# laurits-mumberg/kube-scheduler-simulator-p9

Measured on AMD Instinct MI355X. Metric: filter+score pod x node pairs/sec (5k nodes, Fit+BalancedAllocation), higher is better.
Workload: dtype int64+f64; 1 GPU; cfg2: 5,000 nodes x 10,000 pods, NodeResourcesFit+NodeResourcesBalancedAllocation; nodes_per_gpu=5000, nodes_total=5000, pods=10000, parallelism=1 GPU

## Files before the change

kube-scheduler-simulator-p9_amd/csrc/engine.hip:

```cpp
#include <hip/hip_runtime.h>

#include <algorithm>
#include <cmath>
#include <cstdlib>
#include <cstring>
#include <memory>
#include <string>
#include <vector>
#include <utility>
#include <deque>
#include <atomic>
#include <map>
#include <mutex>
#include <chrono>
#include <cstddef>
#include <thread>

#include "engine.h"
#include <rccl/rccl.h>

namespace ksg {

#define HIPCHK(x)                                                                 \
  do {                                                                            \
// ... 3502 lines not shown
  static_assert(96 * 4 + sizeof(PodLite) + 16 <= 192 * 4, "eval LDS layout");
  auto fetch = [&](uint32_t kk, RowV& r, StaticRec& sr, bool loaded) {
    const uint32_t to = kk * KSG_TILE + tid, nn = tile * A.tile_len + to;
    if (to < A.tile_len && nn < C.N) {
      const int hit = pend_lds((int32_t)(C.goff + nn));
      if (hit >= 0) r = ld_obj<PER>(&A.pprev[hit].after);
      else if (!loaded) load_row_p<PER>(C, nn, A.need_eph, r);
      if (STAT) sr = srec_at<PER>(A, q, C.goff + nn);
    }
  };
  StaticRec snext{KSG_FILTER_PASS, 0};
  fetch(0, rnext, snext, true);
#pragma unroll 1
  for (uint32_t k = 0; k < A.npt; ++k) {
  KSG_ETIME(t0);
  if (A.estamps && w == 15) asm volatile("s_waitcnt vmcnt(0)" ::: "memory");
  KSG_ETIME(tl);
  t_wait += tl - t0;
  const uint32_t to = k * KSG_TILE + tid, n = tile * A.tile_len + to;
  const RowV r = rnext;
  const StaticRec sr = snext;
  if (k + 1 < A.npt) fetch(k + 1, rnext, snext, false);
  uint64_t key = 0;
  bool feasible = false, achT = false, achA = false;
  if (to < A.tile_len && n < C.N) {
    int32_t fit_s, ba_s;
    int64_t total;
    uint32_t code, raw = 0;
    if (STAT) {
      const int64_t MT = mlds[0], MA = mlds[1];
      code = eval_row_s<MODE>(r, F, h, C.R < 4 ? C.R : 4, sr, MT, MA, fit_s, ba_s, total);
      raw = sr.raw;
      achT = F.pos_taint >= 0 && (int64_t)(raw >> 20) == MT;
      achA = F.pos_na >= 0 && !(h->flags & KPF_SKIP_NA_SCORE) && (int64_t)(raw & KSG_RAW_NA_MASK) == MA;
    } else {
      code = eval_row<MODE>(r, F, h, C.R < 4 ? C.R : 4, fit_s, ba_s, total);
    }
    if (stash_all || w == 0) {
      stash[(stash_all ? k * 16 + w : k) * 64 + lane] = PatchV{code, fit_s | (ba_s << 16), (int32_t)total, raw};
    } else {
      uint32_t* of;
      int32_t *os, *ot;
      out_ptrs(A, q, C.N, of, os, ot);
      if (PER && kept_q(A, q)) write_pair<STAT, true>(F, of, os, ot, C.N, n, code, fit_s, ba_s, total, raw);
      else write_pair<STAT, false>(F, of, os, ot, C.N, n, code, fit_s, ba_s, total, raw);
    }
    if (code == KSG_FILTER_PASS) {
      feasible = true;
      key = pack_key(total, F.seed, h->queue_idx, C.goff + n);
    }
  }
  cF += (uint32_t)__popcll(__ballot(feasible));
  if (STAT) {
    cT += (uint32_t)__popcll(__ballot(feasible && achT));
    cA += (uint32_t)__popcll(__ballot(feasible && achA));
  }
  KSG_ETIME(t1);
  key = wave_sort_desc(key);
  top = k == 0 ? key : wave_merge_top(top, wave_reverse(key));
  KSG_ETIME(t2);
  t_eval += t1 - t0;
  t_sort += t2 - t1;
  }
  KSG_ETIME(t3);
  L[w * 64 + lane] = top;
  if (lane == 0) {
    wcount[w] = cF;
    wcount[32 + w] = cT;
    wcount[48 + w] = cA;
  }
  lds_barrier();
#pragma unroll 1
  for (int s = 8; s >= 1; s >>= 1) {
    if (w < s) L[w * 64 + lane] = wave_merge_top(L[w * 64 + lane], L[(w + s) * 64 + 63 - lane]);
    lds_barrier();
  }
  if (w == 0) {
    uint64_t* dst = A.tile_top + ((size_t)b * A.T + tile) * KSG_TOPK;
    __hip_atomic_store(dst + lane, L[lane], __ATOMIC_RELAXED, __HIP_MEMORY_SCOPE_AGENT);
    if (lane < 3) {
      const int off = lane == 0 ? 0 : 16 + 16 * lane;
      int32_t c = 0;
      for (int k = 0; k < 16; ++k) c += (int32_t)wcount[off + k];
      __hip_atomic_store(A.tile_feas + ((size_t)b * A.T + tile) * 3 + lane, c, __ATOMIC_RELAXED,
                         __HIP_MEMORY_SCOPE_AGENT);
    }
    asm volatile("s_waitcnt vmcnt(0)" ::: "memory");
    uint32_t old = 0;
    if (lane == 0) old = __hip_atomic_fetch_add(A.arrive + b * A.astride, 1u, __ATOMIC_RELAXED, __HIP_MEMORY_SCOPE_AGENT);
    old = __builtin_amdgcn_readfirstlane(old);
    if (lane == 0) wcount[16] = old == A.T - 1 ? 1u : 0u;
  }
  auto flush_stash = [&]() {
    if (!stash_all && w != 0) return;
    uint32_t* of;
    int32_t *os, *ot;
    out_ptrs(A, q, C.N, of, os, ot);
#pragma unroll 1
    for (uint32_t k = 0; k < A.npt; ++k) {
      const uint32_t to = k * KSG_TILE + tid, n = tile * A.tile_len + to;
      if (to >= A.tile_len || n >= C.N) break;
      const PatchV pt = stash[(stash_all ? k * 16 + w : k) * 64 + lane];
      if (PER && kept_q(A, q)) write_pair<STAT, true>(F, of, os, ot, C.N, n, pt.code, pt.fitba & 0xFFFF, pt.fitba >> 16, pt.total, pt.raw);
      else write_pair<STAT, false>(F, of, os, ot, C.N, n, pt.code, pt.fitba & 0xFFFF, pt.fitba >> 16, pt.total, pt.raw);
    }
  };
  auto signal_flushed = [&]() {
    if constexpr (PER) {
      asm volatile("s_waitcnt vmcnt(0)" ::: "memory");
      __syncthreads();
      if (tid == 0) __hip_atomic_fetch_add(A.flushed, 1u, __ATOMIC_RELAXED, __HIP_MEMORY_SCOPE_AGENT);
    }
  };
  lds_barrier();
  KSG_ETIME(t4);
#undef KSG_ETIME
  if (est) {
    atomicAdd((unsigned long long*)&A.estamps[13], (unsigned long long)t_eval);
    atomicAdd((unsigned long long*)&A.estamps[14], (unsigned long long)t_sort);
    atomicAdd((unsigned long long*)&A.estamps[15], (unsigned long long)(t4 - t3));
    atomicAdd((unsigned long long*)&A.estamps[18], (unsigned long long)t_wait);
  }
  if (A.estamps && tid == 0) {
    __builtin_amdgcn_sched_barrier(0);
    const uint64_t t = __builtin_amdgcn_s_memrealtime();
    __builtin_amdgcn_sched_barrier(0);
    atomicMax((unsigned long long*)&A.estamps[9], (unsigned long long)t);
    atomicMax((unsigned long long*)&A.estamps[28], (unsigned long long)(t - t_start));
    atomicAdd((unsigned long long*)&A.estamps[29], (unsigned long long)(t - t_start));
    atomicAdd((unsigned long long*)&A.estamps[31], 1ull);
  }
  if (!wcount[16]) {
    flush_stash();
    signal_flushed();
    return;
  }
  win_merge<PER>(C, A, b, L, pnl, np);
  flush_stash();
  signal_flushed();
}

struct SumLite {
  uint64_t best_key;
  int32_t selected, feasible, status, pad;
};
struct Delta {
  int64_t req[4];
  int64_t nzc, nzm;
  int32_t pods;
};
#define KSG_HSLOTS 128
struct PickTab {
  int32_t node[KSG_HSLOTS];
  int32_t first[KSG_HSLOTS], last[KSG_HSLOTS], cnt[KSG_HSLOTS];
};
struct WinLDS {
  uint64_t key[KSG_BATCH][KSG_CAND];
  RowV row[KSG_BATCH][KSG_STAGE];
  Pend prior[KSG_BATCH];
  PodLite pod[KSG_BATCH];
  PatchV patch[KSG_BATCH][KSG_CAND];
  uint64_t pkey[KSG_BATCH][KSG_BATCH];
  int8_t pdf[KSG_BATCH][KSG_BATCH];
  uint64_t pmask[KSG_BATCH];
  uint32_t nxt_ok;
  uint64_t pbest[KSG_BATCH];
  int32_t pbest_e[KSG_BATCH];
  int32_t S[3][KSG_BATCH];
  int32_t O[3][KSG_BATCH];
  int32_t feas[KSG_BATCH];
  SumLite sum[KSG_BATCH];
  int32_t ptn[KSG_HSLOTS], pte[KSG_HSLOTS];
  int32_t gtn[KSG_HSLOTS], gtf[KSG_HSLOTS];
  PickTab pick[3];
  uint64_t kc[KSG_BATCH][KSG_CAND];
  uint64_t rk[KSG_BATCH][KSG_BATCH];
  int8_t rdf[KSG_BATCH][KSG_BATCH];
  int32_t pf[KSG_BATCH];
  int32_t achT[KSG_BATCH], achA[KSG_BATCH];
  int64_t mt[KSG_BATCH], ma[KSG_BATCH];
  int64_t xmt[KSG_BATCH], xma[KSG_BATCH];
  int8_t pdfT[KSG_BATCH][KSG_BATCH], pdfA[KSG_BATCH][KSG_BATCH];
  int8_t rdfT[KSG_BATCH][KSG_BATCH], rdfA[KSG_BATCH][KSG_BATCH];
  int32_t fbf[KSG_BATCH];
  uint64_t red[16][4];
};

static_assert(sizeof(WinLDS) <= 160 * 1024, "window LDS exceeds the CU's 160 KiB");
static constexpr uint32_t kStashNpt =
    (uint32_t)std::min<size_t>(KSG_STASH_NPT, (sizeof(WinLDS) - (16 * 64 * 8 + 192 * 4)) / (16 * 64 * sizeof(PatchV)));
static_assert(kStashNpt >= 1, "eval blocks' output stash exceeds the window LDS");
__device__ __forceinline__ uint32_t hslot(int32_t node) { return ((uint32_t)node * 2654435761u) >> 25; }
__device__ __forceinline__ int prior_of(const WinLDS& L, int32_t x) {
  uint32_t h = hslot(x);
  for (int k = 0; k < KSG_HSLOTS; ++k) {
    int32_t v = L.ptn[h];
    if (v == x) return L.pte[h];
    if (v == -1) return -1;
    h = (h + 1) & (KSG_HSLOTS - 1);
  }
  return -1;
}
__device__ __forceinline__ uint32_t tab_claim(int32_t* nodes, int32_t x) {
  uint32_t h = hslot(x);
  for (int k = 0; k < KSG_HSLOTS; ++k) {
    int32_t old = atomicCAS(&nodes[h], -1, x);
    if (old == -1 || old == x) return h;
    h = (h + 1) & (KSG_HSLOTS - 1);
  }
  return 0;
}
__device__ __forceinline__ int tab_find(const int32_t* nodes, int32_t x) {
  uint32_t h = hslot(x);
  for (int k = 0; k < KSG_HSLOTS; ++k) {
    int32_t v = nodes[h];
    if (v == x) return (int)h;
    if (v == -1) return -1;
    h = (h + 1) & (KSG_HSLOTS - 1);
  }
  return -1;
}
__device__ __forceinline__ void pick_insert(PickTab& T, int32_t x, int b) {
  uint32_t h = tab_claim(T.node, x);
  atomicMin(&T.first[h], b);
  atomicMax(&T.last[h], b);
  atomicAdd(&T.cnt[h], 1);
}
__device__ __forceinline__ void pick_clear(PickTab& T, int i) {
  T.node[i] = -1;
  T.first[i] = KSG_BATCH;
  T.last[i] = -1;
  T.cnt[i] = 0;
}
__device__ __forceinline__ int first_pick(const PickTab& T, int32_t x) {
  int h = x >= 0 ? tab_find(T.node, x) : -1;
  return h >= 0 ? T.first[h] : KSG_BATCH;
}

#define KSG_ORG_NODE 0x40000000
template <bool PER = false>
__device__ __forceinline__ void origin_rows(const DevCluster& C, const WinLDS& L, const WinArgs& A, int32_t o,
                                            RowV& start, RowV& snap) {
  if (o & KSG_ORG_NODE) {
    if (A.xrows) start = A.xrows[o & 0xFFFFF];
    else load_row(C, (uint32_t)(o & 0xFFFFF) - C.goff, A.need_eph, start);
    snap = start;
  } else if (o < KSG_BATCH) {
    start = L.prior[o].after;
    snap = L.prior[o].base;
  } else {
    int p = (o - 64) >> 6, i = (o - 64) & 63;
    if (i < KSG_STAGE) start = L.row[p][i];
    else if (PER) load_row_p<PER>(C, (uint32_t)(L.key[p][i] & 0xFFFFFull) - C.goff, A.need_eph, start);
    else start = rec_rows(A.wrec)[p * KSG_CAND + i];
    snap = start;
  }
}
__device__ __forceinline__ void delta_of(const PodLite& p, Delta& d) {
#pragma unroll
  for (int k = 0; k < 4; ++k) d.req[k] = p.req[k];
  d.nzc = p.nz_cpu;
  d.nzm = p.nz_mem;
  d.pods = 1;
}
__device__ __forceinline__ void delta_add(Delta& d, const PodLite& p) {
#pragma unroll
  for (int k = 0; k < 4; ++k) d.req[k] += p.req[k];
  d.nzc += p.nz_cpu;
  d.nzm += p.nz_mem;
  d.pods += 1;
}
__device__ __forceinline__ void apply_delta(RowV& r, const Delta& d, uint32_t R) {
#pragma unroll
  for (uint32_t k = 0; k < 4; ++k)
    if (k < R) r.req[k] += d.req[k];
  r.nzc += d.nzc;
  r.nzm += d.nzm;
  r.podcnt += d.pods;
}
__device__ __forceinline__ void pick_chain(const WinLDS& L, const int32_t* S, int a, int32_t x, Delta& cum, int& nx) {
  cum = Delta{};
  nx = KSG_BATCH;
  for (int j = 0; j < KSG_BATCH; ++j)
    if (S[j] == x) {
      if (j <= a) delta_add(cum, L.pod[j]);
      else if (nx == KSG_BATCH) nx = j;
    }
}
__device__ __forceinline__ uint64_t max3u(uint64_t a, uint64_t b, uint64_t c) {
  uint64_t m = a > b ? a : b;
  return m > c ? m : c;
}

template <bool PER = false>
__device__ __forceinline__ void row_under(const DevCluster& C, const WinLDS& L, const WinArgs& A, const int32_t* S,
                                          const PickTab& T, int b, uint32_t gu, uint32_t R, RowV& r) {
  const int32_t g = (int32_t)gu;
  const int e = prior_of(L, g);
  if (e >= 0) r = L.prior[e].after;
  else if (A.xrows) r = A.xrows[g];
  else load_row_p<PER>(C, gu - C.goff, A.need_eph, r);
  const int hs = tab_find(T.node, g);
  if (hs >= 0 && T.first[hs] < b) {
    Delta cum{};
    for (int j = 0; j < b; ++j)
      if (S[j] == g) delta_add(cum, L.pod[j]);
    apply_delta(r, cum, R);
  }
}
template <int MODE, bool PER = false>
__device__ __forceinline__ void win_exact_select(const DevCluster& C, const DevProfile& F, const WinArgs& A, WinLDS& L,
                                              int b, int cur, int nxt, uint32_t R) {
  const int tid = threadIdx.x, lane = tid & 63, wave = tid >> 6;
  const PodLite* h = &L.pod[b];
  const int32_t* S = L.S[cur];
  const PickTab& T = L.pick[cur];
  const uint32_t g0 = A.xrows ? 0u : C.goff, gn = A.xrows ? A.G : C.N;
  int32_t feas = 0;
  int64_t lt = 0, la = 0;
#pragma unroll 1
  for (uint32_t i = tid; i < gn; i += KSG_WIN_THREADS) {
    RowV r;
    row_under<PER>(C, L, A, S, T, b, g0 + i, R, r);
    const StaticRec sr = srec_at<PER>(A, A.w0 + b, g0 + i);
    int32_t fs, bs;
    int64_t tot;
    if (eval_row_s<MODE>(r, F, h, R, sr, 0, 0, fs, bs, tot) == KSG_FILTER_PASS) {
      ++feas;
      lt = max(lt, (int64_t)(sr.raw >> 20));
      la = max(la, (int64_t)(sr.raw & KSG_RAW_NA_MASK));
    }
  }
  feas = wave_sum(feas);
  lt = wave_max(lt);
  la = wave_max(la);
  if (lane == 0) {
    L.red[wave][0] = (uint64_t)feas;
    L.red[wave][1] = (uint64_t)lt;
    L.red[wave][2] = (uint64_t)la;
  }
  lds_barrier();
  int32_t fa = 0;
  int64_t mt = 0, ma = 0;
  for (int w = 0; w < KSG_WIN_THREADS / 64; ++w) {
    fa += (int32_t)L.red[w][0];
    mt = max(mt, (int64_t)L.red[w][1]);
    ma = max(ma, (int64_t)L.red[w][2]);
  }
  uint64_t best = 0;
#pragma unroll 1
  for (uint32_t i = tid; i < gn; i += KSG_WIN_THREADS) {
    RowV r;
    row_under<PER>(C, L, A, S, T, b, g0 + i, R, r);
    int32_t fs, bs;
    int64_t tot;
    if (eval_row_s<MODE>(r, F, h, R, srec_at<PER>(A, A.w0 + b, g0 + i), mt, ma, fs, bs, tot) == KSG_FILTER_PASS) {
      const uint64_t k = pack_key(tot, F.seed, h->queue_idx, g0 + i);
      best = k > best ? k : best;
    }
  }
  best = wave_max(best);
  if (lane == 0) L.red[wave][3] = best;
  lds_barrier();
  if (tid == 0) {
    uint64_t bk = 0;
    for (int w = 0; w < KSG_WIN_THREADS / 64; ++w) bk = L.red[w][3] > bk ? L.red[w][3] : bk;
    const int32_t sel = (fa > 0 && bk) ? (int32_t)(bk & 0xFFFFFull) : -1;
    int32_t org = -1;
    if (sel >= 0) {
      const int e = prior_of(L, sel);
      org = e >= 0 ? e : (KSG_ORG_NODE | sel);
      pick_insert(L.pick[nxt], sel, b);
    }
    L.S[nxt][b] = sel;
    L.O[nxt][b] = org;
    SumLite& sm = L.sum[b];
    sm.best_key = sel >= 0 ? (fa == 1 ? (bk & 0xFFFFFFFFFFull) : bk) : 0;
    sm.selected = sel;
    sm.feasible = fa;
    sm.status = sel >= 0 ? 0 : 1;
    L.xmt[b] = mt;
    L.xma[b] = (h->flags & KPF_SKIP_NA_SCORE) ? 0 : ma;
  }
}
template <int MODE, bool PER = false>
__device__ __forceinline__ void win_exact_write(const DevCluster& C, const DevProfile& F, const WinArgs& A, WinLDS& L,
                                             int b, int cur, uint32_t R) {
  const PodLite* h = &L.pod[b];
  uint32_t* of;
  int32_t *os, *ot;
  out_ptrs(A, A.w0 + b, C.N, of, os, ot);
  const int64_t mt = L.xmt[b], ma = L.xma[b];
#pragma unroll 1
  for (uint32_t i = threadIdx.x; i < C.N; i += KSG_WIN_THREADS) {
    RowV r;
    row_under<PER>(C, L, A, L.S[cur], L.pick[cur], b, C.goff + i, R, r);
    const StaticRec sr = srec_at<PER>(A, A.w0 + b, C.goff + i);
    int32_t fs, bs;
    int64_t tot;
    const uint32_t code = eval_row_s<MODE>(r, F, h, R, sr, mt, ma, fs, bs, tot);
    if (PER && kept_q(A, A.w0 + b)) write_pair<true, true>(F, of, os, ot, C.N, i, code, fs, bs, tot, sr.raw);
    else write_pair<true>(F, of, os, ot, C.N, i, code, fs, bs, tot, sr.raw);
  }
}

template <int MODE, bool STAT, bool PER = false>
__device__ __forceinline__ void win_fixup(const DevCluster& C, const DevProfile& F, const WinArgs& A, WinLDS& L) {
  int tid_ = (int)threadIdx.x;
#ifndef KSG_FIXUP_HOIST
  asm volatile("" : "+v"(tid_));
#endif
  const int tid = tid_, lane = tid & 63, wave = tid >> 6;
  const int nb = (int)A.nw;
  const uint32_t R = C.R < 4 ? C.R : 4;
#define STAMP(k)                                        \
  if (A.stamps && tid == 0) {                           \
    __builtin_amdgcn_sched_barrier(0);                  \
    A.stamps[k] = __builtin_amdgcn_s_memtime();         \
    __builtin_amdgcn_sched_barrier(0);                  \
  }
  STAMP(0);
  if (A.stamps && tid == 0) A.stamps[11] = __builtin_amdgcn_s_memrealtime();
  const bool p_late = PER && A.pub_wait != nullptr;
  int np = 0;
  int32_t pn_all = -1;
  uint64_t pv = 0;
  constexpr int kRowW = (int)(sizeof(RowV) / 8), kPendW = (int)(sizeof(Pend) / 8);
  auto p_loads = [&]() {
    np = ldv<PER>(A.pprev_n);
    pn_all = wave == 0 && lane < KSG_BATCH ? ldv<PER>(&A.pprev[lane].node) : -1;
  };
  auto p_list_load = [&]() {
    pv = tid < KSG_BATCH * kPendW ? ldv<PER>(reinterpret_cast<const uint64_t*>(A.pprev) + tid) : 0;
  };
  if (!p_late) p_loads();
  const uint64_t* keys = rec_keys(A.wrec);
  const uint64_t* rows = reinterpret_cast<const uint64_t*>(rec_rows(A.wrec));
  const int nk = nb * KSG_CAND, nr = nb * KSG_STAGE * kRowW;
  uint64_t kv[2], rv[6];
  const ShallowRows* SR = shallow_rows(A.wrec);
// ... 26 lines not shown
    auto small_stores = [&]() {
      if (tid < nb * kPodW) reinterpret_cast<uint64_t*>(L.pod)[tid] = qv;
      if (tid < nb) L.feas[tid] = fv;
      if (STAT && tid < nb) {
        L.achT[tid] = aT;
        L.achA[tid] = aA;
        L.mt[tid] = m0;
        L.ma[tid] = m1;
        L.fbf[tid] = 0;
      }
      if (tid < 3 * KSG_BATCH) {
        (&L.S[0][0])[tid] = -1;
        (&L.O[0][0])[tid] = -1;
      }
      if (tid < KSG_HSLOTS) {
#pragma unroll
        for (int t = 0; t < 3; ++t) pick_clear(L.pick[t], tid);
      }
    };
    if (p_late) small_stores();
    if (p_late) {
      if (tid == 0) {
        bool ok = false;
        if (A.rstamps) A.rstamps[0] = __builtin_amdgcn_s_memrealtime();
        for (uint32_t it = 0; it < A.spin; ++it) {
          if (ld_sc1(A.pub_wait) >= A.pub_wait_need) { ok = true; break; }
          if ((it & 63u) == 63u && ld_sc1(A.abortw) != 0u) break;
          __builtin_amdgcn_s_sleep(1);
        }
        if (A.rstamps) A.rstamps[1] = __builtin_amdgcn_s_memrealtime();
        if (!ok) __hip_atomic_store(A.abortw, 1u, __ATOMIC_RELAXED, __HIP_MEMORY_SCOPE_AGENT);
      }
      lds_barrier();
      p_loads();
      p_list_load();
    }
    if (tid < np * kPendW) reinterpret_cast<uint64_t*>(L.prior)[tid] = pv;
    if (!p_late) small_stores();
    if (wave == 0) {
      const int32_t pnode = lane < np ? pn_all : -1;
      L.ptn[lane] = -1;
      L.ptn[lane + 64] = -1;
      if (lane < np) L.pte[tab_claim(L.ptn, pnode)] = lane;
    }
  }
  lds_barrier();
  STAMP(1);
  if (tid < np) {
    const Pend& pe = L.prior[tid];
    uint32_t nl = (uint32_t)pe.node - C.goff;
    if ((uint32_t)pe.node >= C.goff && nl < C.N) store_row_p<PER>(C, nl, pe.after);
    if (A.xrows) A.xrows[pe.node] = pe.after;
  }
  {
    const int pb = 2 * wave + (lane >> 5), e = lane & 31;
    uint64_t k = 0;
    if (pb < nb && e < np) {
      const Pend& pe = L.prior[e];
      const PodLite* h = &L.pod[pb];
      int32_t fs, bs;
      int64_t tot;
      StaticRec sr{KSG_FILTER_PASS, 0};
      uint32_t code;
      if (STAT) {
        sr = srec_at<PER>(A, A.w0 + pb, (uint32_t)pe.node);
        code = eval_row_s<MODE>(pe.after, F, h, R, sr, L.mt[pb], L.ma[pb], fs, bs, tot);
      } else {
        code = eval_row<MODE>(pe.after, F, h, R, fs, bs, tot);
      }
      bool snap_ok = sr.code == KSG_FILTER_PASS && (F.pos_fit < 0 || fit_filter_row(pe.base, h, R) == 0);
      PatchV pt;
      pt.code = code;
      pt.fitba = fs | (bs << 16);
      pt.total = (int32_t)tot;
      pt.raw = sr.raw;
      L.patch[pb][e] = pt;
      k = code == KSG_FILTER_PASS ? pack_key(tot, F.seed, h->queue_idx, (uint32_t)pe.node) : 0;
      L.pkey[pb][e] = k;
      const int df = (code == KSG_FILTER_PASS ? 1 : 0) - (snap_ok ? 1 : 0);
      L.pdf[pb][e] = (int8_t)df;
      if (STAT) {
        const bool na_on = F.pos_na >= 0 && !(h->flags & KPF_SKIP_NA_SCORE);
        L.pdfT[pb][e] = (int8_t)(F.pos_taint >= 0 && (int64_t)(sr.raw >> 20) == L.mt[pb] ? df : 0);
        L.pdfA[pb][e] = (int8_t)(na_on && (int64_t)(sr.raw & KSG_RAW_NA_MASK) == L.ma[pb] ? df : 0);
      }
    }
    STAMP(16);
    uint64_t k0 = wave_max(lane < 32 ? k : (uint64_t)0), k1 = wave_max(lane >= 32 ? k : (uint64_t)0);
    unsigned long long m0 = __ballot(k0 && lane < 32 && k == k0), m1 = __ballot(k1 && lane >= 32 && k == k1);
    if (lane == 0) {
      if (2 * wave < nb) {
        L.pbest[2 * wave] = k0;
        L.pbest_e[2 * wave] = m0 ? __ffsll((long long)m0) - 1 : -1;
      }
      if (2 * wave + 1 < nb) {
        L.pbest[2 * wave + 1] = k1;
        L.pbest_e[2 * wave + 1] = m1 ? __ffsll((long long)m1) - 1 - 32 : -1;
      }
    }
  }
#pragma unroll
  for (int k = 0; k < 2; ++k) {
    int i = tid + k * KSG_WIN_THREADS;
    if (i < nk) (&L.key[0][0])[i] = kv[k];
    const int b = wave + 16 * k;
    bool m = kv[k] != 0 && np > 0 && prior_of(L, (int32_t)(kv[k] & 0xFFFFFull)) >= 0;
    unsigned long long mask = __ballot(m);
    if (lane == 0 && b < nb) L.pmask[b] = mask;
  }
#pragma unroll
  for (int k = 0; k < 6; ++k) {
    int i = tid + k * KSG_WIN_THREADS;
    if (i < nr) reinterpret_cast<uint64_t*>(&L.row[0][0])[i] = rv[k];
  }
  lds_barrier();
  STAMP(17);
  STAMP(2);
  if (wave == 0) {
    const int b = lane;
    const bool valid = b < nb;
    const uint64_t pm = valid ? L.pmask[b] : 0;
    const uint64_t pbk = valid ? L.pbest[b] : 0;
    int r = 0;
    bool pok = pbk != 0;
    int32_t node = -1, org = -1;
#pragma unroll 1
    for (int round = 0; round < 64; ++round) {
      uint64_t ck = 0;
      if (valid) {
        uint64_t free_ = ~pm & (r < 64 ? (~0ull << r) : 0ull);
        r = free_ ? __ffsll((long long)free_) - 1 : KSG_CAND;
        ck = r < KSG_CAND ? L.key[b][r] : 0;
      }
      uint64_t pk = pok ? pbk : 0;
      uint64_t best = ck > pk ? ck : pk;
      bool from_c = best != 0 && best == ck;
      node = best ? (int32_t)(best & 0xFFFFFull) : -1;
      org = !best ? -1 : from_c ? 64 + b * 64 + r : L.pbest_e[b];
      L.gtn[lane] = -1;
      L.gtn[lane + 64] = -1;
      uint32_t h = 0;
      if (node >= 0) {
        h = tab_claim(L.gtn, node);
        L.gtf[h] = KSG_BATCH;
      }
      if (node >= 0) atomicMin(&L.gtf[h], b);
      bool lose = node >= 0 && L.gtf[h] < b;
      if (__ballot(lose) == 0) break;
      if (lose) {
        if (from_c) ++r;
        else pok = false;
      }
    }
    if (valid) {
      L.S[0][b] = node;
      L.O[0][b] = org;
      if (node >= 0) pick_insert(L.pick[0], node, b);
    }
  }
  lds_barrier();
  STAMP(3);
  int cur = 0, stable = 0;
  uint32_t iters = 0;
#pragma unroll 1
  for (;;) {
    const int nxt = cur == 2 ? 0 : cur + 1;
    if (tid < KSG_HSLOTS) pick_clear(L.pick[nxt == 2 ? 0 : nxt + 1], tid);
    const PickTab& T = L.pick[cur];
    if (wave < 8) {
      const int p_hi = nb * (nb - 1) / 2;
#pragma unroll 1
      for (int base = stable * (stable - 1) / 2 + wave * 64; base < p_hi; base += 8 * 64) {
        const int p = base + lane;
        if (p < p_hi) {
          int b = (int)((1.0f + sqrtf(1.0f + 8.0f * (float)p)) * 0.5f);
          b = b * (b - 1) / 2 > p ? b - 1 : ((b + 1) * b / 2 <= p ? b + 1 : b);
          const int a = p - b * (b - 1) / 2;
          const int32_t Sv = L.S[cur][a];
          uint64_t k = 0;
          int df = 0, dT = 0, dA = 0;
          PatchV pt;
          pt.code = KSG_NOT_PATCHED;
          pt.fitba = pt.total = 0;
          pt.raw = 0;
          if (Sv >= 0) {
            int nx = KSG_BATCH;
            Delta cum;
            delta_of(L.pod[a], cum);
            if (iters == 0) STAMP(24);
            if (T.cnt[tab_find(T.node, Sv)] > 1) pick_chain(L, L.S[cur], a, Sv, cum, nx);
            if (iters == 0) STAMP(25);
            if (nx >= b) {
              RowV cur_r, snap;
              origin_rows<PER>(C, L, A, L.O[cur][a], cur_r, snap);
              apply_delta(cur_r, cum, R);
              const PodLite* h = &L.pod[b];
              int32_t fs, bs;
              int64_t tot;

              StaticRec sr{KSG_FILTER_PASS, 0};
              uint32_t code;
              if (STAT) {
                sr = srec_at<PER>(A, A.w0 + b, (uint32_t)Sv);
                code = eval_row_s<MODE>(cur_r, F, h, R, sr, L.mt[b], L.ma[b], fs, bs, tot);
              } else {
                code = eval_row<MODE>(cur_r, F, h, R, fs, bs, tot);
              }

              bool snap_ok = sr.code == KSG_FILTER_PASS && (F.pos_fit < 0 || fit_filter_row(snap, h, R) == 0);
              df = (code == KSG_FILTER_PASS ? 1 : 0) - (snap_ok ? 1 : 0);
              if (STAT) {
                const bool na_on = F.pos_na >= 0 && !(h->flags & KPF_SKIP_NA_SCORE);
                dT = F.pos_taint >= 0 && (int64_t)(sr.raw >> 20) == L.mt[b] ? df : 0;
                dA = na_on && (int64_t)(sr.raw & KSG_RAW_NA_MASK) == L.ma[b] ? df : 0;
              }
              if (code == KSG_FILTER_PASS) k = pack_key(tot, F.seed, h->queue_idx, (uint32_t)Sv);
              pt.code = code;
              pt.fitba = fs | (bs << 16);
              pt.total = (int32_t)tot;
              pt.raw = sr.raw;
            }
          }
          L.rk[b][a] = k;
          L.rdf[b][a] = (int8_t)df;
          if (STAT) {
            L.rdfT[b][a] = (int8_t)dT;
            L.rdfA[b][a] = (int8_t)dA;
          }
          L.patch[b][32 + a] = pt;
        }
      }
    } else {
      if (wave == 8 && lane < np) L.pf[lane] = first_pick(T, L.prior[lane].node);
#pragma unroll 1
      for (int b = stable + (wave - 8); b < nb; b += 8) {
        const uint64_t ck = L.key[b][lane];
        const bool mod = ((L.pmask[b] >> lane) & 1) || (ck != 0 && first_pick(T, (int32_t)(ck & 0xFFFFFull)) < b);
        L.kc[b][lane] = mod ? 0 : ck;
      }
    }
    if (iters == 0) STAMP(21);
    lds_barrier();
    if (iters == 0) STAMP(22);
#pragma unroll 1
    for (int hh = 0; hh < 2; ++hh) {
      const int b = 2 * wave + hh;
      if (b >= nb) break;
      if (b < stable) {
        if (lane == 0) {
          int32_t s = L.S[cur][b];
          L.S[nxt][b] = s;
          L.O[nxt][b] = L.O[cur][b];
          if (s >= 0) pick_insert(L.pick[nxt], s, b);
        }
        continue;
      }
      const bool pact = lane < np && L.pf[lane & 31] >= b;
      const uint64_t kc = L.kc[b][lane];
      const uint64_t kp = pact ? L.pkey[b][lane & 31] : 0;
      const uint64_t kr = lane < b ? L.rk[b][lane & 31] : 0;
      const int df = (pact ? (int)L.pdf[b][lane & 31] : 0) + (lane < b ? (int)L.rdf[b][lane & 31] : 0);
      const uint64_t best = wave_max(max3u(kc, kp, kr));
      int feasible;
      bool fb = false;
      if (STAT) {
        const int dT = (pact ? (int)L.pdfT[b][lane & 31] : 0) + (lane < b ? (int)L.rdfT[b][lane & 31] : 0);
        const int dA = (pact ? (int)L.pdfA[b][lane & 31] : 0) + (lane < b ? (int)L.rdfA[b][lane & 31] : 0);
        const int sum = wave_sum((df + 2) | ((dT + 2) << 10) | ((dA + 2) << 20));
        feasible = L.feas[b] + (sum & 1023) - 128;
        const int achT = L.achT[b] + ((sum >> 10) & 1023) - 128, achA = L.achA[b] + ((sum >> 20) & 1023) - 128;
        const bool na_on = F.pos_na >= 0 && !(L.pod[b].flags & KPF_SKIP_NA_SCORE);
        fb = !(L.pod[b].flags & KPF_PREFILTER_ERROR) && !na_prescore_error(L.pod[b].flags, feasible) && feasible > 0 &&
             ((F.pos_taint >= 0 && achT <= 0) || (na_on && achA <= 0));
      } else {
        feasible = L.feas[b] + wave_sum(df);
      }
      const bool perr = (L.pod[b].flags & KPF_PREFILTER_ERROR) != 0 || na_prescore_error(L.pod[b].flags, feasible);
      const int32_t sel = (feasible > 0 && best && !perr) ? (int32_t)(best & 0xFFFFFull) : -1;
      const unsigned long long mc = __ballot(best && kc == best), mp = __ballot(best && kp == best),
                               mr = __ballot(best && kr == best);
      if (STAT && lane == 0) L.fbf[b] = fb ? 1 : 0;
      if (fb) continue;
      if (lane == 0) {
        if (STAT) {
          L.xmt[b] = L.mt[b] < 0 ? 0 : L.mt[b];
          L.xma[b] = (F.pos_na < 0 || (L.pod[b].flags & KPF_SKIP_NA_SCORE) || L.ma[b] < 0) ? 0 : L.ma[b];
        }
        int32_t org = -1;
        if (mc) org = 64 + b * 64 + (__ffsll((long long)mc) - 1);
        else if (mp) org = __ffsll((long long)mp) - 1;
        else if (mr) org = L.O[cur][__ffsll((long long)mr) - 1];
        L.S[nxt][b] = sel;
        L.O[nxt][b] = sel >= 0 ? org : -1;
        if (sel >= 0) pick_insert(L.pick[nxt], sel, b);
        SumLite& sm = L.sum[b];
        sm.best_key = sel >= 0 ? (feasible == 1 ? (best & 0xFFFFFFFFFFull) : best) : 0;
        sm.selected = sel;
        sm.feasible = feasible;
        sm.status = perr ? 2 : (sel >= 0 ? 0 : 1);
      }
    }
    if (iters == 0) STAMP(23);
    lds_barrier();
    if (STAT) {
      unsigned long long fm = __ballot(lane < nb && lane >= stable && L.fbf[lane & 31] != 0);
      if (fm) {
        while (fm) {
          const int b = __ffsll((long long)fm) - 1;
          fm &= fm - 1;
          win_exact_select<MODE, PER>(C, F, A, L, b, cur, nxt, R);
        }
        lds_barrier();
      }
    }
    if (iters < 2) STAMP(19 + iters);
    ++iters;
    {
      const int32_t so = L.S[cur][lane & 31], sn = L.S[nxt][lane & 31];
      unsigned long long m = __ballot(lane < nb && lane >= stable && sn != so);
      stable = m ? min(__ffsll((long long)m), nb) : nb;
    }
    cur = nxt;
    if (stable >= nb) break;
  }
  STAMP(4);
  if (A.stamps && tid == 0) A.stamps[7] = iters;
  uint32_t pre_fl = 0, pre_ev = 0;
  if (PER && tid == 0) {
    pre_fl = ld_sc1(A.flushed);
    pre_ev = A.nxt_evd ? ld_sc1(A.nxt_evd) : 0u;
  }
  auto flushed_wait = [&]() {
    if (tid == 0) {
      bool ok = pre_fl >= A.flush_need;
      for (uint32_t it = 0; !ok && it < A.spin; ++it) {
        if (ld_sc1(A.flushed) >= A.flush_need) { ok = true; break; }
        if ((it & 63u) == 63u && ld_sc1(A.abortw) != 0u) break;
        __builtin_amdgcn_s_sleep(2);
      }
      if (!ok) __hip_atomic_store(A.abortw, 1u, __ATOMIC_RELAXED, __HIP_MEMORY_SCOPE_AGENT);
    }
    lds_barrier();
  };
  auto exact_writes = [&]() {
    unsigned long long fm = __ballot(lane < nb && L.fbf[lane & 31] != 0);
    while (fm) {
      const int b = __ffsll((long long)fm) - 1;
      fm &= fm - 1;
      win_exact_write<MODE, PER>(C, F, A, L, b, cur, R);
    }
  };
  bool exact_early = false;
  if constexpr (PER && STAT) {
    if (A.replay2 && __ballot(lane < nb && L.fbf[lane & 31] != 0) != 0) {
      exact_early = true;
      flushed_wait();
      exact_writes();
    }
  }
  const PickTab& T = L.pick[cur];
  if (wave == 0) {
    const int a = lane;
    const int32_t Sv = a < nb ? L.S[cur][a] : -1;
    int h = Sv >= 0 ? tab_find(T.node, Sv) : -1;
    const bool last = h >= 0 && T.last[h] == a;
    unsigned long long m = __ballot(last);
    if (last) {
      Delta cum;
      delta_of(L.pod[a], cum);
      int nx;
      if (T.cnt[h] > 1) pick_chain(L, L.S[cur], a, Sv, cum, nx);
      RowV st, snap;
      origin_rows<PER>(C, L, A, L.O[cur][a], st, snap);
      Pend p;
      p.node = Sv;
      p.pad = 0;
      p.base = st;
      apply_delta(st, cum, R);
      p.after = st;
      st_obj<PER>(A.pnext + __popcll(m & ((1ull << a) - 1)), p);
    }
    if (lane == 0) stv<PER>(A.pnext_n, (int32_t)__popcll(m));
  }
  STAMP(26);
  if constexpr (PER) {
    asm volatile("s_waitcnt vmcnt(0)" ::: "memory");
    STAMP(27);
    __syncthreads();
    if (tid < 16) {
      if (A.replay2) __hip_atomic_fetch_max(A.pub + tid * 32, A.pub_val, __ATOMIC_RELAXED, __HIP_MEMORY_SCOPE_AGENT);
      else st_sc1(A.pub + tid * 32, A.pub_val);
    }
    if (A.rstamps && tid == 0) A.rstamps[2] = __builtin_amdgcn_s_memrealtime();
  }
  STAMP(6);
  if (tid < nb) {
    ksg_pod_summary& d = A.sums[A.w0 + tid];
    d.best_key = L.sum[tid].best_key;
    d.selected = L.sum[tid].selected;
    d.feasible = L.sum[tid].feasible;
    d.status = L.sum[tid].status;
    if (STAT) {
      if (F.pos_taint >= 0) d.max_score[F.pos_taint] = L.xmt[tid];
      if (F.pos_na >= 0) d.max_score[F.pos_na] = L.xma[tid];
    }
  }
  if constexpr (PER) {
    if (tid == 0) L.nxt_ok = A.nxt_evd && pre_ev >= A.nxt_need ? 1u : 0u;
    if (!exact_early) flushed_wait();
  }
  {
    const int32_t Sv = L.S[cur][lane & 31];
    const int32_t pn = lane < np ? L.prior[lane].node : -1;
    const int pf = lane < np ? first_pick(T, pn) : -1;
#pragma unroll 1
    for (int hh = 0; hh < 2; ++hh) {
      const int b = 2 * wave + hh;
      if (b >= nb) break;
      if (STAT && L.fbf[b]) continue;
      const PatchV pt = L.patch[b][lane];
      const bool wr = lane < 32 ? (lane < np && pf >= b) : (lane - 32 < b && pt.code != KSG_NOT_PATCHED);
      const int32_t node = lane < 32 ? pn : Sv;
      const uint32_t nl = (uint32_t)node - C.goff;
      if (wr && node >= 0 && (uint32_t)node >= C.goff && nl < C.N) {
        uint32_t* of;
        int32_t *os, *ot;
        out_ptrs(A, A.w0 + b, C.N, of, os, ot);
        if (PER && kept_q(A, A.w0 + b))
          write_pair<STAT, true>(F, of, os, ot, C.N, nl, pt.code, pt.fitba & 0xFFFF, pt.fitba >> 16, pt.total, pt.raw);
        else
          write_pair<STAT, false>(F, of, os, ot, C.N, nl, pt.code, pt.fitba & 0xFFFF, pt.fitba >> 16, pt.total, pt.raw);
      }
    }
  }
  if (STAT && !exact_early) exact_writes();
  STAMP(5);
  if (A.stamps && tid == 0) A.stamps[12] = __builtin_amdgcn_s_memrealtime();
#undef STAMP
}

template <int MODE, bool STAT>
__global__ __launch_bounds__(KSG_WIN_THREADS) void k_window(DevCluster C, DevProfile F, WinArgs A) {
  extern __shared__ __attribute__((aligned(16))) unsigned char lds_raw[];
  uint32_t warm = 0;
  KWarm<0, (int)((sizeof(DevCluster) + sizeof(DevProfile) + sizeof(WinArgs)) / 64 * 64)>::run(
      (const void*)__builtin_amdgcn_kernarg_segment_ptr(), warm);
  warm_wait(warm);
  if (blockIdx.x == 0) {
    if (A.nw) win_fixup<MODE, STAT>(C, F, A, *reinterpret_cast<WinLDS*>(lds_raw));
    return;
  }
  win_eval<MODE, STAT>(C, F, A, blockIdx.x - 1, reinterpret_cast<uint64_t*>(lds_raw));
}

__global__ void k_apply_pend(DevCluster C, const Pend* p, const int32_t* pn) {
  int e = threadIdx.x;
  if (e >= *pn) return;
  uint32_t nl = (uint32_t)p[e].node - C.goff;
  if ((uint32_t)p[e].node >= C.goff && nl < C.N) store_row(C, nl, p[e].after);
}

__global__ __launch_bounds__(64) void k_window_gmerge(const uint8_t* recv, uint32_t ranks, const RowV* xrows,
                                                      const Pend* pl, const int32_t* pn, uint8_t* out) {
  __shared__ uint64_t keys[8 * KSG_CAND];
  const uint32_t b = blockIdx.x;
  const int lane = threadIdx.x;
  for (uint32_t r = 0; r < ranks; ++r) keys[r * KSG_CAND + lane] = rec_keys(recv + r * kXchgBytes)[(size_t)b * KSG_CAND + lane];
  __syncthreads();
  uint64_t v = keys[lane];
  for (uint32_t r = 1; r < ranks; ++r) v = wave_merge_top(v, keys[r * KSG_CAND + 63 - lane]);
  int32_t f[3] = {0, 0, 0};
  for (uint32_t r = 0; r < ranks; ++r)
    for (int k = 0; k < 3; ++k) f[k] += reinterpret_cast<const int32_t*>(recv + r * kXchgBytes)[k * KSG_BATCH + b];
  RowV c;
  memset(&c, 0, sizeof(c));
  if (v) {
    const int32_t gid = (int32_t)(v & 0xFFFFFull);
    const int np = *pn;
    int hit = -1;
    for (int e = 0; e < np; ++e) hit = pl[e].node == gid ? e : hit;
    c = hit >= 0 ? pl[hit].after : xrows[gid];
  }
  rec_keys(out)[(size_t)b * KSG_CAND + lane] = v;
  rec_rows(out)[(size_t)b * KSG_CAND + lane] = c;
  if (lane < 3) reinterpret_cast<int32_t*>(out)[lane * KSG_BATCH + b] = f[lane];
}
__global__ void k_rows_pack(DevCluster C, uint32_t need_eph, RowV* out) {
  const uint32_t n = blockIdx.x * blockDim.x + threadIdx.x;
  if (n < C.N) load_row(C, n, need_eph, out[n]);
}
__global__ void k_rows_unpack(const RowV* recv, uint32_t ranks, uint32_t G, uint32_t stride, RowV* xrows) {
  const uint32_t r = blockIdx.y;
  const uint32_t lo = (uint32_t)((uint64_t)G * r / ranks), hi = (uint32_t)((uint64_t)G * (r + 1) / ranks);
  for (uint32_t i = blockIdx.x * blockDim.x + threadIdx.x; lo + i < hi; i += gridDim.x * blockDim.x)
    xrows[lo + i] = recv[(size_t)r * stride + i];
}

#include "table_chain.hip"

struct WinSync {
  uint32_t replayed[16][32];
  uint32_t evd[2];
  uint32_t pad1[30];
  uint32_t flushed[2];
  uint32_t pad2[30];
};
struct WinRunArgs {
  uint32_t nwin, first, count, T;
  uint32_t tt_sz, tf_sz;
  uint64_t* tile_top;
  int32_t* tfeas;
  uint8_t* wrec;
  Pend* pend;
  int32_t* pend_n;
  uint32_t* arrive;
  uint64_t* stamps;
  const uint32_t* sready;
  uint32_t sready_need;
};
__device__ bool win_stat_gate(const WinRunArgs& R, uint32_t r0, uint32_t n, uint32_t* abortw, uint32_t spin,
                              uint32_t* go) {
  if (threadIdx.x == 0) {
    const uint32_t g0 = r0 / KSG_SD_PODS, g1 = (r0 + n - 1) / KSG_SD_PODS;
    bool ok = false;
    for (uint32_t it = 0; it < spin; ++it) {
      bool all = true;
      for (uint32_t g = g0; g <= g1; ++g) all &= ld_sc1(R.sready + g) >= R.sready_need;
      if (all) { ok = true; break; }
      if ((it & 63u) == 63u && ld_sc1(abortw) != 0u) break;
      __builtin_amdgcn_s_sleep(2);
    }
    if (!ok) __hip_atomic_store(abortw, 1u, __ATOMIC_RELAXED, __HIP_MEMORY_SCOPE_AGENT);
// ... 3170 lines not shown
```

Baseline: 8.209 billion pairs/s.

## Cache per-pick base/after rows in LDS across fixpoint iterations

Adds a per-batch PickRow cache in LDS holding base, after and snap rows plus the next-pick index for each selected node. Each pairwise conflict evaluation and the final pending-row output now read these cached rows instead of rebuilding them through origin_rows and pick_chain on every pair. The change also drops the last/cnt atomics from the pick table, specializes the non-STAT selection path with paired wave reductions, and exits the loop early once no selection changes. In exchange it costs extra LDS space and a fill pass with a barrier each iteration, and the deep-origin handling adds subtle invariants that could break correctness.

```diff
diff --git a/kube-scheduler-simulator-p9_amd/csrc/engine.hip b/kube-scheduler-simulator-p9_amd/csrc/engine.hip
--- a/kube-scheduler-simulator-p9_amd/csrc/engine.hip
+++ b/kube-scheduler-simulator-p9_amd/csrc/engine.hip
@@ -3678,7 +3678,15 @@
 #define KSG_HSLOTS 128
 struct PickTab {
   int32_t node[KSG_HSLOTS];
-  int32_t first[KSG_HSLOTS], last[KSG_HSLOTS], cnt[KSG_HSLOTS];
+  int32_t first[KSG_HSLOTS];
+};
+struct PickRow {
+  RowV base;
+  RowV after;
+  RowV snap;
+  int32_t node;
+  int32_t nx;
+  int32_t deep, pad;
 };
 struct WinLDS {
   uint64_t key[KSG_BATCH][KSG_CAND];
@@ -3699,6 +3707,7 @@
   int32_t ptn[KSG_HSLOTS], pte[KSG_HSLOTS];
   int32_t gtn[KSG_HSLOTS], gtf[KSG_HSLOTS];
   PickTab pick[3];
+  PickRow pr[KSG_BATCH];
   uint64_t kc[KSG_BATCH][KSG_CAND];
   uint64_t rk[KSG_BATCH][KSG_BATCH];
   int8_t rdf[KSG_BATCH][KSG_BATCH];
@@ -3749,14 +3758,10 @@
 __device__ __forceinline__ void pick_insert(PickTab& T, int32_t x, int b) {
   uint32_t h = tab_claim(T.node, x);
   atomicMin(&T.first[h], b);
-  atomicMax(&T.last[h], b);
-  atomicAdd(&T.cnt[h], 1);
 }
 __device__ __forceinline__ void pick_clear(PickTab& T, int i) {
   T.node[i] = -1;
   T.first[i] = KSG_BATCH;
-  T.last[i] = -1;
-  T.cnt[i] = 0;
 }
 __device__ __forceinline__ int first_pick(const PickTab& T, int32_t x) {
   int h = x >= 0 ? tab_find(T.node, x) : -1;
@@ -3804,14 +3809,38 @@
   r.nzm += d.nzm;
   r.podcnt += d.pods;
 }
-__device__ __forceinline__ void pick_chain(const WinLDS& L, const int32_t* S, int a, int32_t x, Delta& cum, int& nx) {
-  cum = Delta{};
-  nx = KSG_BATCH;
-  for (int j = 0; j < KSG_BATCH; ++j)
-    if (S[j] == x) {
-      if (j <= a) delta_add(cum, L.pod[j]);
-      else if (nx == KSG_BATCH) nx = j;
-    }
+template <bool PER>
+__device__ __forceinline__ void win_fill_rows(const DevCluster& C, WinLDS& L, const WinArgs& A, const int32_t* S,
+                                              const int32_t* O, int nb, int keep, uint32_t R, int tid) {
+  const int a = tid >> 5, j = tid & 31;
+  const int32_t Sa = S[a], Sj = S[j];
+  PickRow& e = L.pr[a];
+  const bool same = e.node == Sa;
+  const uint32_t m = (uint32_t)(__ballot(Sa >= 0 && Sj == Sa) >> (tid & 32));
+  if (a >= nb || j > 2) return;
+  if (j == 0) {
+    const uint32_t later = a < KSG_BATCH - 1 ? m & (~0u << (a + 1)) : 0u;
+    e.nx = later ? __ffs((int)later) - 1 : KSG_BATCH;
+    e.node = Sa;
+    e.deep = 0;
+  }
+  if (Sa < 0 || (same && a < keep)) return;
+  RowV st, snap;
+  if (same) {
+    st = e.base;
+    snap = e.snap;
+  } else {
+    origin_rows<PER>(C, L, A, O[a], st, snap);
+  }
+  if (j == 0) {
+    Delta cum{};
+    for (uint32_t le = m & (~0u >> (KSG_BATCH - 1 - a)); le; le &= le - 1) delta_add(cum, L.pod[__ffs((int)le) - 1]);
+    apply_delta(st, cum, R);
+    e.after = st;
+  } else if (!same) {
+    if (j == 1) e.base = st;
+    else e.snap = snap;
+  }
 }
 __device__ __forceinline__ uint64_t max3u(uint64_t a, uint64_t b, uint64_t c) {
   uint64_t m = a > b ? a : b;
@@ -4144,10 +4173,27 @@
         else pok = false;
       }
     }
-    if (valid) {
-      L.S[0][b] = node;
-      L.O[0][b] = org;
+    if (lane < KSG_BATCH) {
+      PickRow& e = L.pr[b];
+      e.node = node;
+      e.nx = KSG_BATCH;
+      if (valid) {
+        L.S[0][b] = node;
+        L.O[0][b] = org;
+      }
+      const bool deep = node >= 0 && org >= 64 && ((org - 64) & 63) >= KSG_STAGE;
+      e.deep = deep ? 1 : 0;
       if (node >= 0) pick_insert(L.pick[0], node, b);
+      if (node >= 0 && !deep) {
+        RowV st, snap;
+        origin_rows<PER>(C, L, A, org, st, snap);
+        e.base = st;
+        e.snap = snap;
+        Delta d;
+        delta_of(L.pod[b], d);
+        apply_delta(st, d, R);
+        e.after = st;
+      }
     }
   }
   lds_barrier();
@@ -4161,6 +4207,17 @@
     const PickTab& T = L.pick[cur];
     if (wave < 8) {
       const int p_hi = nb * (nb - 1) / 2;
+      if (iters == 0 && tid == 8 * 64 - 1 && L.pr[nb - 1].deep) {
+        PickRow& e = L.pr[nb - 1];
+        RowV st, snap;
+        origin_rows<PER>(C, L, A, L.O[cur][nb - 1], st, snap);
+        e.base = st;
+        e.snap = snap;
+        Delta d;
+        delta_of(L.pod[nb - 1], d);
+        apply_delta(st, d, R);
+        e.after = st;
+      }
 #pragma unroll 1
       for (int base = stable * (stable - 1) / 2 + wave * 64; base < p_hi; base += 8 * 64) {
         const int p = base + lane;
@@ -4168,7 +4225,8 @@
           int b = (int)((1.0f + sqrtf(1.0f + 8.0f * (float)p)) * 0.5f);
           b = b * (b - 1) / 2 > p ? b - 1 : ((b + 1) * b / 2 <= p ? b + 1 : b);
           const int a = p - b * (b - 1) / 2;
-          const int32_t Sv = L.S[cur][a];
+          PickRow& e = L.pr[a];
+          const int32_t Sv = e.node;
           uint64_t k = 0;
           int df = 0, dT = 0, dA = 0;
           PatchV pt;
@@ -4176,16 +4234,25 @@
           pt.fitba = pt.total = 0;
           pt.raw = 0;
           if (Sv >= 0) {
-            int nx = KSG_BATCH;
-            Delta cum;
-            delta_of(L.pod[a], cum);
             if (iters == 0) STAMP(24);
-            if (T.cnt[tab_find(T.node, Sv)] > 1) pick_chain(L, L.S[cur], a, Sv, cum, nx);
+            const int nx = e.nx;
             if (iters == 0) STAMP(25);
             if (nx >= b) {
               RowV cur_r, snap;
-              origin_rows<PER>(C, L, A, L.O[cur][a], cur_r, snap);
-              apply_delta(cur_r, cum, R);
+              if (e.deep) {
+                origin_rows<PER>(C, L, A, L.O[cur][a], cur_r, snap);
+                if (b == a + 1) {
+                  e.base = cur_r;
+                  e.snap = snap;
+                }
+                Delta d;
+                delta_of(L.pod[a], d);
+                apply_delta(cur_r, d, R);
+                if (b == a + 1) e.after = cur_r;
+              } else {
+                cur_r = e.after;
+                snap = e.snap;
+              }
               const PodLite* h = &L.pod[b];
               int32_t fs, bs;
               int64_t tot;
@@ -4234,62 +4301,119 @@
     if (iters == 0) STAMP(21);
     lds_barrier();
     if (iters == 0) STAMP(22);
+    if constexpr (STAT) {
 #pragma unroll 1
-    for (int hh = 0; hh < 2; ++hh) {
-      const int b = 2 * wave + hh;
-      if (b >= nb) break;
-      if (b < stable) {
+      for (int hh = 0; hh < 2; ++hh) {
+        const int b = 2 * wave + hh;
+        if (b >= nb) break;
+        if (b < stable) {
+          if (lane == 0) {
+            int32_t s = L.S[cur][b];
+            L.S[nxt][b] = s;
+            L.O[nxt][b] = L.O[cur][b];
+            if (s >= 0) pick_insert(L.pick[nxt], s, b);
+          }
+          continue;
+        }
+        const bool pact = lane < np && L.pf[lane & 31] >= b;
+        const uint64_t kc = L.kc[b][lane];
+        const uint64_t kp = pact ? L.pkey[b][lane & 31] : 0;
+        const uint64_t kr = lane < b ? L.rk[b][lane & 31] : 0;
+        const int df = (pact ? (int)L.pdf[b][lane & 31] : 0) + (lane < b ? (int)L.rdf[b][lane & 31] : 0);
+        const uint64_t best = wave_max(max3u(kc, kp, kr));
+        const int dT = (pact ? (int)L.pdfT[b][lane & 31] : 0) + (lane < b ? (int)L.rdfT[b][lane & 31] : 0);
+        const int dA = (pact ? (int)L.pdfA[b][lane & 31] : 0) + (lane < b ? (int)L.rdfA[b][lane & 31] : 0);
+        const int sum = wave_sum((df + 2) | ((dT + 2) << 10) | ((dA + 2) << 20));
+        const int feasible = L.feas[b] + (sum & 1023) - 128;
+        const int achT = L.achT[b] + ((sum >> 10) & 1023) - 128, achA = L.achA[b] + ((sum >> 20) & 1023) - 128;
+        const bool na_on = F.pos_na >= 0 && !(L.pod[b].flags & KPF_SKIP_NA_SCORE);
+        const bool fb = !(L.pod[b].flags & KPF_PREFILTER_ERROR) && !na_prescore_error(L.pod[b].flags, feasible) &&
+                        feasible > 0 && ((F.pos_taint >= 0 && achT <= 0) || (na_on && achA <= 0));
+        const bool perr = (L.pod[b].flags & KPF_PREFILTER_ERROR) != 0 || na_prescore_error(L.pod[b].flags, feasible);
+        const int32_t sel = (feasible > 0 && best && !perr) ? (int32_t)(best & 0xFFFFFull) : -1;
+        const unsigned long long mc = __ballot(best && kc == best), mp = __ballot(best && kp == best),
+                                 mr = __ballot(best && kr == best);
+        if (lane == 0) L.fbf[b] = fb ? 1 : 0;
+        if (fb) continue;
         if (lane == 0) {
+          L.xmt[b] = L.mt[b] < 0 ? 0 : L.mt[b];
+          L.xma[b] = (F.pos_na < 0 || (L.pod[b].flags & KPF_SKIP_NA_SCORE) || L.ma[b] < 0) ? 0 : L.ma[b];
+          int32_t org = -1;
+          if (mc) org = 64 + b * 64 + (__ffsll((long long)mc) - 1);
+          else if (mp) org = __ffsll((long long)mp) - 1;
+          else if (mr) org = L.O[cur][__ffsll((long long)mr) - 1];
+          L.S[nxt][b] = sel;
+          L.O[nxt][b] = sel >= 0 ? org : -1;
+          if (sel >= 0) pick_insert(L.pick[nxt], sel, b);
+          SumLite& sm = L.sum[b];
+          sm.best_key = sel >= 0 ? (feasible == 1 ? (best & 0xFFFFFFFFFFull) : best) : 0;
+          sm.selected = sel;
+          sm.feasible = feasible;
+          sm.status = perr ? 2 : (sel >= 0 ? 0 : 1);
+        }
+      }
+    } else {
+      const int b0 = 2 * wave;
+      uint64_t kc[2], kp[2], kr[2], best[2];
+      int pk[2], sum[2];
+#pragma unroll
+      for (int hh = 0; hh < 2; ++hh) {
+        const int b = b0 + hh;
+        const bool pact = lane < np && L.pf[lane & 31] >= b;
+        kc[hh] = L.kc[b][lane];
+        kp[hh] = pact ? L.pkey[b][lane & 31] : 0;
+        kr[hh] = lane < b ? L.rk[b][lane & 31] : 0;
+        const int df = (pact ? (int)L.pdf[b][lane & 31] : 0) + (lane < b ? (int)L.rdf[b][lane & 31] : 0);
+        pk[hh] = df;
+      }
+      {
+        const uint64_t m0 = max3u(kc[0], kp[0], kr[0]), m1 = max3u(kc[1], kp[1], kr[1]);
+        const uint32_t h0 = (uint32_t)(m0 >> 32), h1 = (uint32_t)(m1 >> 32);
+        const uint32_t mh0 = __ockl_wfred_max_u32(h0), mh1 = __ockl_wfred_max_u32(h1);
+        const uint32_t ml0 = __ockl_wfred_max_u32(h0 == mh0 ? (uint32_t)m0 : 0u),
+                       ml1 = __ockl_wfred_max_u32(h1 == mh1 ? (uint32_t)m1 : 0u);
+        sum[0] = wave_sum(pk[0]);
+        sum[1] = wave_sum(pk[1]);
+        best[0] = ((uint64_t)mh0 << 32) | ml0;
+        best[1] = ((uint64_t)mh1 << 32) | ml1;
+      }
+      unsigned long long mc[2], mp[2], mr[2];
+#pragma unroll
+      for (int hh = 0; hh < 2; ++hh) {
+        mc[hh] = __ballot(best[hh] && kc[hh] == best[hh]);
+        mp[hh] = __ballot(best[hh] && kp[hh] == best[hh]);
+        mr[hh] = __ballot(best[hh] && kr[hh] == best[hh]);
+      }
+      const int hh = lane >> 5, b = b0 + hh;
+      if ((lane & 31) == 0 && b < nb) {
+        if (b < stable) {
           int32_t s = L.S[cur][b];
           L.S[nxt][b] = s;
           L.O[nxt][b] = L.O[cur][b];
           if (s >= 0) pick_insert(L.pick[nxt], s, b);
+        } else {
+          const uint64_t bk = hh ? best[1] : best[0];
+          const unsigned long long c = hh ? mc[1] : mc[0], p = hh ? mp[1] : mp[0], r = hh ? mr[1] : mr[0];
+          const int sm_ = hh ? sum[1] : sum[0];
+          const uint32_t fl = L.pod[b].flags;
+          const int feasible = L.feas[b] + sm_;
+          {
+            const bool perr = (fl & KPF_PREFILTER_ERROR) != 0 || na_prescore_error(fl, feasible);
+            const int32_t sel = (feasible > 0 && bk && !perr) ? (int32_t)(bk & 0xFFFFFull) : -1;
+            int32_t org = -1;
+            if (c) org = 64 + b * 64 + (__ffsll((long long)c) - 1);
+            else if (p) org = __ffsll((long long)p) - 1;
+            else if (r) org = L.O[cur][__ffsll((long long)r) - 1];
+            L.S[nxt][b] = sel;
+            L.O[nxt][b] = sel >= 0 ? org : -1;
+            if (sel >= 0) pick_insert(L.pick[nxt], sel, b);
+            SumLite& sm = L.sum[b];
+            sm.best_key = sel >= 0 ? (feasible == 1 ? (bk & 0xFFFFFFFFFFull) : bk) : 0;
+            sm.selected = sel;
+            sm.feasible = feasible;
+            sm.status = perr ? 2 : (sel >= 0 ? 0 : 1);
+          }
         }
-        continue;
-      }
-      const bool pact = lane < np && L.pf[lane & 31] >= b;
-      const uint64_t kc = L.kc[b][lane];
-      const uint64_t kp = pact ? L.pkey[b][lane & 31] : 0;
-      const uint64_t kr = lane < b ? L.rk[b][lane & 31] : 0;
-      const int df = (pact ? (int)L.pdf[b][lane & 31] : 0) + (lane < b ? (int)L.rdf[b][lane & 31] : 0);
-      const uint64_t best = wave_max(max3u(kc, kp, kr));
-      int feasible;
-      bool fb = false;
-      if (STAT) {
-        const int dT = (pact ? (int)L.pdfT[b][lane & 31] : 0) + (lane < b ? (int)L.rdfT[b][lane & 31] : 0);
-        const int dA = (pact ? (int)L.pdfA[b][lane & 31] : 0) + (lane < b ? (int)L.rdfA[b][lane & 31] : 0);
-        const int sum = wave_sum((df + 2) | ((dT + 2) << 10) | ((dA + 2) << 20));
-        feasible = L.feas[b] + (sum & 1023) - 128;
-        const int achT = L.achT[b] + ((sum >> 10) & 1023) - 128, achA = L.achA[b] + ((sum >> 20) & 1023) - 128;
-        const bool na_on = F.pos_na >= 0 && !(L.pod[b].flags & KPF_SKIP_NA_SCORE);
-        fb = !(L.pod[b].flags & KPF_PREFILTER_ERROR) && !na_prescore_error(L.pod[b].flags, feasible) && feasible > 0 &&
-             ((F.pos_taint >= 0 && achT <= 0) || (na_on && achA <= 0));
-      } else {
-        feasible = L.feas[b] + wave_sum(df);
-      }
-      const bool perr = (L.pod[b].flags & KPF_PREFILTER_ERROR) != 0 || na_prescore_error(L.pod[b].flags, feasible);
-      const int32_t sel = (feasible > 0 && best && !perr) ? (int32_t)(best & 0xFFFFFull) : -1;
-      const unsigned long long mc = __ballot(best && kc == best), mp = __ballot(best && kp == best),
-                               mr = __ballot(best && kr == best);
-      if (STAT && lane == 0) L.fbf[b] = fb ? 1 : 0;
-      if (fb) continue;
-      if (lane == 0) {
-        if (STAT) {
-          L.xmt[b] = L.mt[b] < 0 ? 0 : L.mt[b];
-          L.xma[b] = (F.pos_na < 0 || (L.pod[b].flags & KPF_SKIP_NA_SCORE) || L.ma[b] < 0) ? 0 : L.ma[b];
-        }
-        int32_t org = -1;
-        if (mc) org = 64 + b * 64 + (__ffsll((long long)mc) - 1);
-        else if (mp) org = __ffsll((long long)mp) - 1;
-        else if (mr) org = L.O[cur][__ffsll((long long)mr) - 1];
-        L.S[nxt][b] = sel;
-        L.O[nxt][b] = sel >= 0 ? org : -1;
-        if (sel >= 0) pick_insert(L.pick[nxt], sel, b);
-        SumLite& sm = L.sum[b];
-        sm.best_key = sel >= 0 ? (feasible == 1 ? (best & 0xFFFFFFFFFFull) : best) : 0;
-        sm.selected = sel;
-        sm.feasible = feasible;
-        sm.status = perr ? 2 : (sel >= 0 ? 0 : 1);
       }
     }
     if (iters == 0) STAMP(23);
@@ -4307,12 +4431,17 @@
     }
     if (iters < 2) STAMP(19 + iters);
     ++iters;
+    bool changed;
     {
       const int32_t so = L.S[cur][lane & 31], sn = L.S[nxt][lane & 31];
       unsigned long long m = __ballot(lane < nb && lane >= stable && sn != so);
       stable = m ? min(__ffsll((long long)m), nb) : nb;
+      changed = m != 0;
     }
     cur = nxt;
+    if (!changed) break;
+    win_fill_rows<PER>(C, L, A, L.S[cur], L.O[cur], nb, stable, R, tid);
+    lds_barrier();
     if (stable >= nb) break;
   }
   STAMP(4);
@@ -4353,23 +4482,15 @@
   const PickTab& T = L.pick[cur];
   if (wave == 0) {
     const int a = lane;
-    const int32_t Sv = a < nb ? L.S[cur][a] : -1;
-    int h = Sv >= 0 ? tab_find(T.node, Sv) : -1;
-    const bool last = h >= 0 && T.last[h] == a;
+    const PickRow& e = L.pr[a & 31];
+    const bool last = a < nb && e.node >= 0 && e.nx == KSG_BATCH;
     unsigned long long m = __ballot(last);
     if (last) {
-      Delta cum;
-      delta_of(L.pod[a], cum);
-      int nx;
-      if (T.cnt[h] > 1) pick_chain(L, L.S[cur], a, Sv, cum, nx);
-      RowV st, snap;
-      origin_rows<PER>(C, L, A, L.O[cur][a], st, snap);
       Pend p;
-      p.node = Sv;
+      p.node = e.node;
       p.pad = 0;
-      p.base = st;
-      apply_delta(st, cum, R);
-      p.after = st;
+      p.base = e.base;
+      p.after = e.after;
       st_obj<PER>(A.pnext + __popcll(m & ((1ull << a) - 1)), p);
     }
     if (lane == 0) stv<PER>(A.pnext_n, (int32_t)__popcll(m));
```

New measurement: 8.847 billion pairs/s (median of 6 runs). 7.8% higher.
